# RKWin93/E2E-MAPPO-for-MT-FJSP

Measured on NVIDIA B200. Metric: MT-FJSP env-steps/sec, higher is better.
Workload: dtype f64

## Files before the change

e2e-mappo-for-mt-fjsp_b200/_lib.py:

```python
from __future__ import annotations

import ctypes as C
import os
import subprocess

_HERE = os.path.dirname(os.path.abspath(__file__))
SRC_DIR = os.path.join(_HERE, "csrc")
LIB_PATH = os.environ.get("MTFJSP_LIB") or os.path.join(_HERE, "libmtfjsp_b200.so")
HEADER = os.path.join(os.path.dirname(_HERE), "include", "mtfjsp.h")
SOURCES = ["mtfjsp_env.cu", "mtfjsp_encoder.cu", "mtfjsp_gemm.cu"]
NVCC_FLAGS = ["-gencode", "arch=compute_100a,code=sm_100a", "-O3", "-lineinfo", "-std=c++17", "-Xcompiler", "-fPIC"]
EXTRA_FLAGS = {"mtfjsp_env.cu": ["-fmad=false"]}


def _stale() -> bool:
    if not os.path.exists(LIB_PATH):
        return True
    mt = os.path.getmtime(LIB_PATH)
    deps = [os.path.join(SRC_DIR, s) for s in os.listdir(SRC_DIR)] + [HEADER, os.path.abspath(__file__)]
    return any(os.path.getmtime(d) > mt for d in deps)


def build(force: bool = False, verbose: bool = False) -> str:
    if force or _stale():
# ... 51 lines not shown
    "mtfjsp_enc_mach_proj": ([_VP, _VP, _VP, _VP, _VP, C.c_int64, _VP], _I),
    "mtfjsp_enc_gat_attend": ([_VP, _VP, _VP, _VP, C.c_int64, _I, _VP], _I),
    "mtfjsp_enc_gat_attend_bwd": ([_VP, _VP, _VP, _VP, _VP, _VP, C.c_int64, _I, _VP], _I),
    "mtfjsp_enc_gat_attend_bwd_blocks": ([C.c_int64], _I),
    "mtfjsp_enc_bias_tanh": ([_VP, _VP, C.c_int64, _I, C.c_int64, _VP], _I),
    "mtfjsp_enc_tanh_dot": ([_VP, _VP, _VP, _VP, C.c_int64, _VP], _I),
    "mtfjsp_enc_gat_trunk_tf32": ([_VP, _VP, _VP, _VP, _VP, _VP, _VP, _VP, _VP, C.c_int64, _VP], _I),
    "mtfjsp_enc_aggregate_linear_tf32": ([_VP, C.c_int64, _I, _VP, _VP, _VP, _VP, _VP, _VP, _I, _VP, _VP, _VP], _I),
    "mtfjsp_enc_select": ([_VP, _VP, _VP, C.c_float, _I, C.c_int64, _I, _U64, _VP, _I, _VP, _VP, _VP, _VP, _VP], _I),
    "mtfjsp_enc_head_tf32": ([_VP, _VP, C.c_int64, _I, _I, _VP, _VP, _I, _VP, _VP, C.c_int64, _VP, _VP, _VP, _VP, _VP, _VP], _I),
    "mtfjsp_enc_wgrad_tf32": ([_VP, _VP, C.c_int64, _I, _VP, _VP, _VP, _VP], _I),
    "mtfjsp_enc_wgrad_workspace_floats": ([_I], C.c_int64),
    "mtfjsp_enc_bn_finalize": ([_VP, C.c_int64, _VP, _VP, C.c_float, _VP, _VP, _I, _VP], _I),
    "mtfjsp_gae4": ([_VP, _VP, _VP, _VP, _VP, _VP, _I, C.c_int64, C.c_float, C.c_float, _VP], _I),
    "mtfjsp_adv_normalize": ([_VP, _VP, C.c_double, _I, C.c_int64, _VP], _I),
    "mtfjsp_launch_count": ([_VP], C.c_int64),
    "mtfjsp_bytes_per_step": ([_VP, _I], C.c_int64),
    "mtfjsp_bytes_per_random_step": ([_VP, _I], C.c_int64),
    "mtfjsp_random_step_is_fused": ([_VP], _I),
    "mtfjsp_last_error": ([], C.c_char_p),
    "mtfjsp_version": ([], C.c_char_p),
}


def lib():
    global _lib
    if _lib is None:
        if not os.path.exists(LIB_PATH):
            raise RuntimeError(
                "CUDA extension %s is missing; run `python -c 'import __graft_entry__ as g; g.build()'` "
# ... 17 lines not shown
```

e2e-mappo-for-mt-fjsp_b200/csrc/mtfjsp_env.cu:

```cuda
#include <assert.h>
#include <cuda_runtime.h>
#include <math.h>
#include <stdint.h>
#include <stdio.h>
#include <stdlib.h>
#include <string.h>

#include <new>
#include <vector>

#include "../../include/mtfjsp.h"

#define MAX_LEAVES 64
#define MAX_PROG 128
#define FULL 0xffffffffu

namespace {

struct Layout {
    int B, J, M, N, E, left_shift;
    int sd_stride, si_stride, xs_stride;
    int o_st, o_ft, o_dur, o_psel, o_scal, o_macc, o_w, o_eacc, o_eleaf, o_ipre, nich, o_sc;
    int o_mach, o_ord, o_rpred, o_cnt, o_misc, o_nxt;
    int o_mind, o_minpt, o_tt;
// ... 38 lines not shown
    unsigned char* rec;
    int rec_stride;
    int b0, b1;
    int rev;
    void* tfea;
    void* mfea;
    float* adj_w;
    int16_t* adj_src;
    uint8_t* jmask;
    int32_t* cand;
    int mask_mode;
    int obs_inc;
    uint8_t* jm_fin;
    uint8_t* jm_esa;
    int32_t* cand_int;
};

enum { MODE_STEP = 1, MODE_OBS = 2, MODE_RESET = 4, MODE_POLICY = 8,
       MODE_HOST = 16,
       MODE_FROM_RESET = 32 };

#define INFO6_PUT(b_, k_, v_)                                                                               \
    do {                                                                                                    \
        if (P.info6) P.info6[(size_t)(b_) * 6 + (k_)] = (v_);                                               \
        if (P.rec) {                                                                                        \
            unsigned char* r_ = P.rec + (size_t)(b_) * P.rec_stride;                                        \
            if ((k_) == 1) r_[REC_DONE] = (v_) != 0.0 ? 1 : 0;                                              \
            else reinterpret_cast<double*>(r_)[(k_) == 0 ? 0 : (k_) - 1] = (v_);                            \
        }                                                                                                   \
    } while (0)
// ... 580 lines not shown
#define MTFJSP_SPEC_TTG 0
#endif
    static constexpr bool TTG = MTFJSP_SPEC_TTG && !NOTT && G_ == 8 && minb(NPT_CHUNK, 0) > minb(NPT_FULL, BTT_FULL) &&
                                minb(NPT_CHUNK, 0) > minb(NPT_CHUNK, BTT_FULL);
    static constexpr int B_TT = TTG ? 0 : BTT_FULL;
    static constexpr bool CHUNK = COLD_ || TTG || minb(NPT_CHUNK, B_TT) > minb(NPT_FULL, B_TT);
    static constexpr int NPT = CHUNK ? NPT_CHUNK : NPT_FULL;
    static_assert(NPT >= 3 * M, "the random-step mode parks three compacted machine rows in the idle-term scratch");
    static constexpr int B_PT = NPT * 8;
    static constexpr int RAW = calign(B_SD + B_TT + B_PT + B_SI, 16);
    static constexpr int ENV_BYTES = env_bytes(NPT, B_TT);
    static constexpr bool BAR_IN_PAD = ENV_BYTES - RAW >= 8;
    static constexpr int ITER = (N + G - 1) / G;
    static constexpr unsigned GMASK = (G_ == 32) ? 0xffffffffu : ((1u << G_) - 1u);
    static constexpr int MINB = minb(NPT, B_TT);
};

__device__ __forceinline__ void bulk_g2s(void* smem_dst, const void* gmem_src, uint32_t bytes, uint32_t bar) {
    const uint32_t d = (uint32_t)__cvta_generic_to_shared(smem_dst);
    asm volatile("cp.async.bulk.shared::cluster.global.mbarrier::complete_tx::bytes [%0], [%1], %2, [%3];" ::"r"(d),
                 "l"(gmem_src), "r"(bytes), "r"(bar)
                 : "memory");
}

template <int G>
__device__ __forceinline__ double gmax_d(double v) {
#pragma unroll
    for (int o = G / 2; o > 0; o >>= 1) v = fmax(v, __shfl_xor_sync(FULL, v, o));
    return v;
}
// ... 32 lines not shown
        double r = 0.0;
        for (int i = 0; i < n; i++) r += a[i];
        return r;
    }
    double r[8];
    for (int i = 0; i < 8; i++) r[i] = a[i];
    int nb = n - (n & 7), i;
    for (i = 8; i < nb; i += 8)
        for (int k = 0; k < 8; k++) r[k] += a[i + k];
    double res = ((r[0] + r[1]) + (r[2] + r[3])) + ((r[4] + r[5]) + (r[6] + r[7]));
    for (; i < n; i++) res += a[i];
    return res;
}

__device__ __forceinline__ int kth_set_bit(unsigned bits, int k, int ) { return (int)__fns(bits, 0u, k + 1); }

template <class S, int MODE, typename OutT>
__global__ void __launch_bounds__(S::WARPS * 32, S::MINB) env_kernel_s(const __grid_constant__ Params P) {
    constexpr int J = S::J, M = S::M, N = S::N, G = S::G, EPW = S::EPW, ITER = S::ITER;
    extern __shared__ __align__(16) unsigned char smem_raw[];
    const int lane = threadIdx.x & 31, warp = threadIdx.x >> 5;
    const int gl = lane & (G - 1), ge = lane / G;
    const unsigned gmask = S::GMASK << (ge * G);
    const int B = P.b1;
    const int blk = P.rev ? (int)(gridDim.x - 1 - blockIdx.x) : (int)blockIdx.x;
    const int wb0 = P.b0 + (blk * S::WARPS + warp) * EPW;
    if (wb0 >= B) return;
    const int b = wb0 + ge;
    const bool active = b < B;
    const int bc = active ? b : wb0;

    unsigned char* base = smem_raw + (size_t)(warp * EPW + ge) * S::ENV_BYTES;
    double* s_sd = reinterpret_cast<double*>(base);
    const double* __restrict__ s_tt = reinterpret_cast<const double*>(base + S::B_SD);
    double* __restrict__ s_pt = reinterpret_cast<double*>(base + S::B_SD + S::B_TT);
    int16_t* __restrict__ s_si = reinterpret_cast<int16_t*>(base + S::B_SD + S::B_TT + S::B_PT);
    constexpr int RECW = rec_bytes(J) / 8, MBYTES = (J + 7) / 8;
    static_assert(6 + RECW - 5 <= S::NPT, "step info and record tail are staged in the idle-term scratch");
    unsigned char* const s_rec = reinterpret_cast<unsigned char*>(s_pt + 6) - REC_DONE;
    constexpr bool REC_STAGED = (MODE & MODE_HOST) != 0;
#define INFO6_S(k_, v_)                                                                      \
// ... 14 lines not shown
    const double* g_xs = P.xs + (size_t)bc * S::XS;
    constexpr bool fr = (MODE & MODE_FROM_RESET) != 0;
    static_assert(!fr || (!S::COLD && (MODE & MODE_STEP)), "COLD reads dur / psel from the state record, not the snapshot");
#ifdef MTFJSP_DEBUG_BOUNDS
    if (fr) assert(bc < P.L.B && P.L.sd_stride == S::SD && P.L.si_stride == S::SI);
#endif
    const double* src_sd = fr ? P.sd0 + (size_t)bc * S::SD : g_sd;
    const int16_t* src_si = fr ? P.si0 + (size_t)bc * S::SI : g_si;

    int a = 0, m = 0;
    bool sel = false;
    int cj = 0;
    int nsel_step = 0;
    int eid = 0;
    if constexpr ((MODE & MODE_POLICY) != 0) {
        const uint8_t* jsrc = (P.mask_mode == MTFJSP_MASK_ESA ? P.jm_esa : P.jm_fin) + (size_t)bc * J;
        if (gl < J) {
            sel = fr ? true : jsrc[gl] == 0;
            cj = fr ? gl * M : P.cand_int[(size_t)bc * J + gl];
        }
        if (gl < M && P.mfea1 != nullptr) eid = __ldg(P.edge_id + (size_t)bc * M + gl);
        nsel_step = fr ? 0 : g_si[S::O_MISC + 2];
    } else if (MODE & MODE_STEP) {
        if (P.act2) { const int2 am = __ldg(P.act2 + bc); a = am.x; m = am.y; }
        else { a = __ldg(P.op + bc); m = __ldg(P.mach + bc); }
    }
    uint64_t* s_bar = S::BAR_IN_PAD
                          ? reinterpret_cast<uint64_t*>(smem_raw + (size_t)(warp * EPW) * S::ENV_BYTES + S::RAW)
                          : reinterpret_cast<uint64_t*>(smem_raw + (size_t)S::WARPS * EPW * S::ENV_BYTES) + warp;
    const uint32_t bar = (uint32_t)__cvta_generic_to_shared(s_bar);
    if (lane == 0) {
        asm volatile("mbarrier.init.shared::cta.b64 [%0], 1;" ::"r"(bar));
        asm volatile("fence.mbarrier_init.release.cluster;" ::: "memory");
        asm volatile("mbarrier.arrive.expect_tx.shared::cta.b64 _, [%0], %1;" ::"r"(bar),
                     "r"((uint32_t)(EPW * (S::SM_SD * 8 + S::B_TT + S::SI * 2 + (fr ? (S::SD - (S::O_SC & ~1)) * 8 : 0))))
                     : "memory");
    }
    __syncwarp();
    if (gl == 0) {
        if constexpr (S::COLD) {
            bulk_g2s(s_sd, g_sd, S::HOT * 8, bar);
            bulk_g2s(s_sd + S::HOT, g_sd + 4 * N, S::TAILBLK * 8, bar);
        } else {
            bulk_g2s(s_sd, src_sd, S::SD * 8, bar);
        }
        if constexpr (S::B_TT > 0) bulk_g2s(base + S::B_SD, g_xs + S::O_TT, S::TT * 8, bar);
        bulk_g2s(s_si, src_si, S::SI * 2, bar);
    }
    constexpr int SC0 = S::O_SC & ~1;
    static_assert(S::NPT >= S::SD - SC0, "the scaler block is staged in the idle-term scratch");
    double wv = 0.0;
    if constexpr (fr) {
        if (gl == 0) bulk_g2s(s_pt, g_sd + SC0, (S::SD - SC0) * 8, bar);
        if (gl < 3) wv = P.weights[(size_t)bc * 3 + gl];
    }
    if constexpr (S::TTG) {
        if (gl < 4) {
            const int o = gl * 16 < M * M - 1 ? gl * 16 : M * M - 1;
            asm volatile("prefetch.global.L1 [%0];" ::"l"(g_xs + S::O_TT + o));
        }
    }
// ... 643 lines not shown
            }
            if (P.mfea && gl < M && active) emit_mach(gl, c > 0 ? (int)s_ord[incs - 1] : 0);
        }
    }

    if (fr && active) {
        const double2* s2 = reinterpret_cast<const double2*>(s_sd);
        double2* g2 = reinterpret_cast<double2*>(g_sd);
#pragma unroll 1
        for (int i = gl; i < S::SD / 2; i += G) g2[i] = s2[i];
        const int4* s4 = reinterpret_cast<const int4*>(s_si);
        int4* g4 = reinterpret_cast<int4*>(g_si);
#pragma unroll 1
        for (int i = gl; i < S::SI / 8; i += G) g4[i] = s4[i];
    }
}

__global__ void load_kernel(Layout L, const double* __restrict__ t, const double* __restrict__ p,
                            const double* __restrict__ tt, const int32_t* __restrict__ edge, int W, double* xs,
                            int8_t* edge_id) {
    size_t gid = (size_t)blockIdx.x * blockDim.x + threadIdx.x;
    size_t total = (size_t)L.B * L.N;
    if (gid < total) {
        size_t b = gid / L.N;
        int i = (int)(gid % L.N);
        const double* tr = t + gid * L.M;
        const double* pr = p + gid * L.M;
        double mn = INFINITY, mnpt = INFINITY;
        for (int m = 0; m < L.M; m++) {
            double tv = tr[m], ptv = tv * fabs(pr[m]);
// ... 447 lines not shown
    int rec_stride;
    uint8_t *dn, *inv;
    float* tmp_adj_w;
    int16_t* tmp_adj_src;
    bool loaded, reset_done, force_generic;
    bool obs_inc_enabled, obs_inc_allowed, obs_synced;
    const void* obs_ptrs[4];
    int obs_dtype;
    int host_zerocopy;
    int host_chunks, fuse_policy;
    int alternate_order, flip;
    unsigned char* slab;
    size_t slab_bytes, window_bytes;
    int l2_persist;
    int64_t launches;
    struct HostPipe* pipe;
};

struct HostPipe {
    static constexpr int MAXC = 8;
    cudaStream_t ms, cs[MAXC];
    cudaEvent_t fork, join[MAXC], hev[MAXC], kev[MAXC];
    struct Entry {
        const void* key[11];
        int mask_mode, dtype, chunks, kernels, inc;
        cudaGraphExec_t exec;
    };
    std::vector<Entry> cache;
};

// ... 6 lines not shown
static Params make_params(mtfjsp_env* h) {
    Params P;
    memset(&P, 0, sizeof P);
    P.L = h->L;
    P.pw = h->pw;
    P.sd = h->sd; P.si = h->si; P.xs = h->xs; P.t = h->t; P.p = h->p;
    P.cfgw[0] = h->cfgw[0]; P.cfgw[1] = h->cfgw[1]; P.cfgw[2] = h->cfgw[2];
    P.divisor = h->divisor; P.gamma = h->gamma;
    P.jm_fin = h->jm_fin; P.jm_esa = h->jm_esa; P.cand_int = h->cand;
    P.b0 = 0; P.b1 = h->L.B;
    return P;
}

static int flush_reset(mtfjsp_env* h, cudaStream_t s) {
    const Layout& L = h->L;
    if (h->pend_reset) {
        reset_copy_kernel<<<L.B, 128, 0, s>>>(L, h->sd0, h->si0, h->pend_w, h->sd, h->si, h->jm_fin, h->jm_esa, h->cand);
        h->launches++;
        h->pend_reset = false;
        CK(cudaGetLastError(), "reset_copy_kernel");
    }
    if (h->pend_scaler) {
        const size_t n = (size_t)L.B * 4;
        scaler_kernel<<<(unsigned)((n + 255) / 256), 256, 0, s>>>(L, h->sd, 0);
        h->launches++;
        h->pend_scaler = false;
        CK(cudaGetLastError(), "scaler_kernel");
    }
    return MTFJSP_OK;
}

static int enter(mtfjsp_env* h, cudaStream_t s, bool step = false) {
    CK(cudaSetDevice(h->device), "cudaSetDevice");
    return step ? MTFJSP_OK : flush_reset(h, s);
}

template <int MODE, typename OutT>
static int launch_env(mtfjsp_env* h, const Params& P, cudaStream_t s) {
    const Layout& L = h->L;
    int rc = flush_reset(h, s);
    if (rc != MTFJSP_OK) return rc;
    size_t smem = (size_t)L.smem_per_warp * L.warps_per_block;
    static thread_local int configured_dev = -1;
    static thread_local size_t configured_smem = 0;
    if (configured_dev != h->device || configured_smem < smem) {
        CK(cudaFuncSetAttribute(env_kernel<MODE, OutT>, cudaFuncAttributeMaxDynamicSharedMemorySize, (int)smem),
           "cudaFuncSetAttribute");
        configured_dev = h->device;
        configured_smem = smem;
    }
    int blocks = (P.b1 - P.b0 + L.warps_per_block - 1) / L.warps_per_block;
    env_kernel<MODE, OutT><<<blocks, L.warps_per_block * 32, smem, s>>>(P);
    h->launches++;
    CK(cudaGetLastError(), "env_kernel launch");
    return MTFJSP_OK;
}

template <class S, int MODE, typename OutT>
static int launch_spec(mtfjsp_env* h, const Params& P, cudaStream_t s) {
    const Layout& L = h->L;
    if (L.sd_stride != S::SD || L.si_stride != S::SI || L.xs_stride != S::XS || L.o_sc != S::O_SC || L.o_misc != S::O_MISC ||
        L.o_eacc != S::O_EACC || L.o_eleaf != S::O_ELEAF || L.o_ipre != S::O_IPRE || L.nich != S::NICH || h->pw.nleaves != S::NLEAF)
        return fail(MTFJSP_E_STATE, "specialised kernel layout mismatch");
    if constexpr (!S::COLD && (MODE & MODE_STEP) && !(MODE & (MODE_HOST | MODE_FROM_RESET))) {
        if (h->pend_reset) {
            Params Q = P;
            Q.sd0 = h->sd0; Q.si0 = h->si0; Q.weights = h->pend_w; Q.clear_ret = h->pend_scaler ? 1 : 0;
            h->pend_reset = h->pend_scaler = false;
// ... 7 lines not shown
    static const size_t extra = getenv("MTFJSP_EXTRA_SMEM") ? (size_t)atoi(getenv("MTFJSP_EXTRA_SMEM")) : 0;
    const size_t smem = (size_t)S::WARPS * S::EPW * S::ENV_BYTES + (S::BAR_IN_PAD ? 0 : 16 * ((S::WARPS * 8 + 15) / 16)) + extra;
    static thread_local int configured_dev = -1;
    if (configured_dev != h->device) {
        CK(cudaFuncSetAttribute(env_kernel_s<S, MODE, OutT>, cudaFuncAttributeMaxDynamicSharedMemorySize, (int)smem),
           "cudaFuncSetAttribute");
        configured_dev = h->device;
    }
    const int per_block = S::WARPS * S::EPW;
    const int blocks = (P.b1 - P.b0 + per_block - 1) / per_block;
    Params Q = P;
    if (h->alternate_order && (MODE & MODE_STEP)) {
        Q.rev = h->flip;
        h->flip ^= 1;
    }
    if (h->window_bytes && (MODE & MODE_STEP)) {
        cudaLaunchConfig_t cfg = {};
        cfg.gridDim = dim3(blocks);
        cfg.blockDim = dim3(S::WARPS * 32);
        cfg.dynamicSmemBytes = smem;
        cfg.stream = s;
        cudaLaunchAttribute at[1];
        at[0].id = cudaLaunchAttributeAccessPolicyWindow;
        at[0].val.accessPolicyWindow.base_ptr = h->slab;
        at[0].val.accessPolicyWindow.num_bytes = h->window_bytes;
        at[0].val.accessPolicyWindow.hitRatio = 1.0f;
        at[0].val.accessPolicyWindow.hitProp = cudaAccessPropertyPersisting;
        at[0].val.accessPolicyWindow.missProp = cudaAccessPropertyStreaming;
        cfg.attrs = at;
        cfg.numAttrs = 1;
        CK(cudaLaunchKernelEx(&cfg, env_kernel_s<S, MODE, OutT>, Q), "env_kernel_s launch");
    } else {
        env_kernel_s<S, MODE, OutT><<<blocks, S::WARPS * 32, smem, s>>>(Q);
    }
    h->launches++;
    CK(cudaGetLastError(), "env_kernel_s launch");
    return MTFJSP_OK;
}

#define MTFJSP_SPEC_SIZES(X) \
    X(6, 6, 8, 4, false) X(10, 6, 16, 1, false) X(20, 6, 32, 1, false) X(10, 10, 16, 1, false) X(15, 10, 32, 1, true) \
    X(20, 10, 32, 1, true) X(30, 20, 32, 1, true)

static int envs_per_wave(int J, int M, int device) {
    int sms = 0;
    if (cudaDeviceGetAttribute(&sms, cudaDevAttrMultiProcessorCount, device) != cudaSuccess || sms <= 0) return 0;
#define X(JJ, MM, GG, WW, CC) \
    if (J == JJ && M == MM) return sms * Spec<JJ, MM, GG, WW, CC>::MINB * WW * Spec<JJ, MM, GG, WW, CC>::EPW;
    MTFJSP_SPEC_SIZES(X)
#undef X
    return 0;
// ... 141 lines not shown
    L.smem_per_warp = align_up(off, 16);
    int wpb = 8;
    while (wpb > 1 && (size_t)wpb * L.smem_per_warp > 200 * 1024) wpb >>= 1;
    if ((size_t)wpb * L.smem_per_warp > 227 * 1024) { delete h; return fail(MTFJSP_E_ARG, "instance too large for shared memory"); }
    L.warps_per_block = wpb;
    h->device = device;
    {
        const char* fg = getenv("MTFJSP_FORCE_GENERIC");
        h->force_generic = fg && fg[0] == '1';
        h->host_chunks = getenv("MTFJSP_HOST_CHUNKS") ? atoi(getenv("MTFJSP_HOST_CHUNKS")) : 4;
        h->host_zerocopy = getenv("MTFJSP_HOST_ZEROCOPY") ? atoi(getenv("MTFJSP_HOST_ZEROCOPY")) : (B >= 16384 ? 2 : 1);
        h->fuse_policy = getenv("MTFJSP_FUSE_POLICY") ? atoi(getenv("MTFJSP_FUSE_POLICY")) : 1;
        h->alternate_order = getenv("MTFJSP_ALTERNATE_ORDER") ? atoi(getenv("MTFJSP_ALTERNATE_ORDER")) : 1;
        h->obs_inc_allowed = !(getenv("MTFJSP_OBS_INCREMENTAL") && atoi(getenv("MTFJSP_OBS_INCREMENTAL")) == 0);
        h->fused_reset = getenv("MTFJSP_FUSED_RESET") ? atoi(getenv("MTFJSP_FUSED_RESET")) : 1;
    }
    h->cfgw[0] = 0.4; h->cfgw[1] = 0.4; h->cfgw[2] = 0.2; h->divisor = 1.0; h->gamma = 0.99;
    size_t Bs = (size_t)B;
#define ALLOC(ptr, bytes)                                                      \
    do {                                                                       \
        cudaError_t e_ = cudaMalloc((void**)&(ptr), (bytes));                  \
        if (e_ != cudaSuccess) { mtfjsp_destroy(h); return fail(MTFJSP_E_CUDA, "cudaMalloc", e_); } \
        cudaMemset((ptr), 0, (bytes));                                         \
    } while (0)
    ALLOC(h->sd, Bs * L.sd_stride * 8);
    {
        auto up = [](size_t x) { return (x + 255) / 256 * 256; };
        const size_t b_si = up(Bs * L.si_stride * 2), b_jm = up(Bs * J), b_cd = up(Bs * J * 4), b_xs = up(Bs * L.xs_stride * 8);
        h->slab_bytes = b_si + 2 * b_jm + b_cd + b_xs;
        ALLOC(h->slab, h->slab_bytes);
// ... 23 lines not shown
    ALLOC(h->edge_id, Bs * M);
    ALLOC(h->a_op, Bs * 4);
    ALLOC(h->a_mach, Bs * 4);
    ALLOC(h->r5, Bs * 5 * 8);
    ALLOC(h->s4, Bs * 4 * 8);
    ALLOC(h->info6, Bs * 6 * 8);
    h->rec_stride = rec_bytes(J);
    ALLOC(h->act2, Bs * 8);
    ALLOC(h->rec, Bs * h->rec_stride);
    ALLOC(h->dn, Bs);
    ALLOC(h->inv, Bs);
    ALLOC(h->tmp_adj_w, Bs * N * 2 * 4);
    ALLOC(h->tmp_adj_src, Bs * N * 2);
    ALLOC(h->sd0, Bs * L.sd_stride * 8);
    ALLOC(h->si0, Bs * L.si_stride * 2);
#undef ALLOC
    *out = h;
    return MTFJSP_OK;
}

int mtfjsp_destroy(mtfjsp_env* h) {
    if (!h) return MTFJSP_OK;
    cudaSetDevice(h->device);
    void* ptrs[] = {h->sd, h->slab, h->t, h->p, h->edge_id, h->a_op, h->a_mach,
                    h->r5, h->s4, h->info6, h->dn, h->inv, h->tmp_adj_w, h->tmp_adj_src, h->act2, h->rec, h->sd0, h->si0};
    for (void* q : ptrs)
        if (q) cudaFree(q);
    if (h->pipe) {
        for (auto& e : h->pipe->cache) cudaGraphExecDestroy(e.exec);
        cudaStreamDestroy(h->pipe->ms);
        cudaEventDestroy(h->pipe->fork);
        for (int c = 0; c < HostPipe::MAXC; c++) {
            cudaStreamDestroy(h->pipe->cs[c]); cudaEventDestroy(h->pipe->join[c]);
            cudaEventDestroy(h->pipe->hev[c]); cudaEventDestroy(h->pipe->kev[c]);
        }
        delete h->pipe;
    }
    delete h;
    return MTFJSP_OK;
}

int mtfjsp_set_params(mtfjsp_env* h, double w_mk, double w_ec, double w_tt, double scaling_divisor, double gamma) {
// ... 509 lines not shown
    return host_step_impl(h, io, task_fea, mach_fea, adj_w, adj_src, mask_mode, dtype, (cudaStream_t)stream);
}

int mtfjsp_step_host_packed(mtfjsp_env* h, const int32_t* actions_host, void* records_host, void* task_fea, void* mach_fea,
                            float* adj_w, int16_t* adj_src, int mask_mode, int dtype, void* stream) {
    if (!h || !actions_host || !records_host) return fail(MTFJSP_E_ARG, "mtfjsp_step_host_packed: bad argument");
    if (!h->reset_done) return fail(MTFJSP_E_STATE, "mtfjsp_step_host_packed before mtfjsp_reset");
    int rc = enter(h, (cudaStream_t)stream);
    if (rc) return rc;
    HostIO io = {nullptr, nullptr, actions_host, nullptr, nullptr, nullptr, (unsigned char*)records_host};
    return host_step_impl(h, io, task_fea, mach_fea, adj_w, adj_src, mask_mode, dtype, (cudaStream_t)stream);
}

int mtfjsp_host_record_bytes(const mtfjsp_env* h) { return h ? h->rec_stride : 0; }

int64_t mtfjsp_launch_count(const mtfjsp_env* h) { return h ? h->launches : 0; }

int64_t mtfjsp_bytes_per_step(const mtfjsp_env* h, int dtype) {
    if (!h) return 0;
    const int64_t N = h->L.N, M = h->L.M, J = h->L.J;
    int64_t b_state = 18 * N + 42 * M + 8 * J + (N + 7) / 8 + 160;
    int64_t fe = dtype == MTFJSP_F64 ? 8 : 4;
    int64_t b_out = 12 * fe * N + 18 * N + 8 * fe * M + 5 * J + 41;
    return 8 + 2 * b_state + b_out;
}

int64_t mtfjsp_bytes_per_random_step(const mtfjsp_env* h, int dtype) {
    if (!h) return 0;
    const int64_t M = h->L.M, J = h->L.J;
    const int64_t fe = dtype == MTFJSP_F64 ? 8 : 4;
// ... 10 lines not shown
```

e2e-mappo-for-mt-fjsp_b200/env.py:

```python
from __future__ import annotations

import ctypes as C

import numpy as np
import torch

from . import _lib
from ._lib import check

F32, F64 = 0, 1
MASK_FINISHED, MASK_ESA = 0, 1


def _ptr(t):
    return None if t is None else C.c_void_p(t.data_ptr())


def _stream():
    return C.c_void_p(torch.cuda.current_stream().cuda_stream)


def _to_dev(x, device, dtype):
    if not torch.is_tensor(x):
        x = torch.as_tensor(np.ascontiguousarray(x))
# ... 192 lines not shown
        return dict(mach=mach, st=st, ft=ft, routes=routes)

    def export_scaler(self):
        dev, B = self.device, self.B
        R = torch.empty((B, 4), dtype=torch.float64, device=dev)
        mean = torch.empty_like(R)
        S = torch.empty_like(R)
        n = torch.empty((B,), dtype=torch.int64, device=dev)
        check(self._lib.mtfjsp_export_scaler(self._h, _ptr(R), _ptr(mean), _ptr(S), _ptr(n), _stream()), "mtfjsp_export_scaler")
        return dict(R=R, mean=mean, S=S, n=n)

    @property
    def launch_count(self):
        return int(self._lib.mtfjsp_launch_count(self._h))

    def bytes_per_step(self):
        return int(self._lib.mtfjsp_bytes_per_step(self._h, self._dt))

    def bytes_per_random_step(self):
        return int(self._lib.mtfjsp_bytes_per_random_step(self._h, self._dt))

    @property
    def random_step_is_fused(self):
        return bool(self._lib.mtfjsp_random_step_is_fused(self._h))
```

e2e-mappo-for-mt-fjsp_b200/parallel_env.py:

```python
from __future__ import annotations

import random

import numpy as np
import torch

from .env import MASK_ESA, MASK_FINISHED, BatchedMTFJSPEnv


def draw_reward_weights(kind: str, configs: dict):
    if kind == "01":
        w = np.array([random.uniform(0, 1) for _ in range(3)])
        return w / np.sum(w, axis=-1)
    if kind == "0.1":
        nums = [round(random.uniform(0, 1), 1) for _ in range(3)]
        total = sum(nums)
        return np.array([round(x / total, 1) for x in nums])
    if kind == "eval":
        return np.array([configs["weight_mk"], configs["weight_ec"], configs["weight_tt"]], dtype=np.float64)
    raise ValueError("Random_weight_type must be '01', '0.1' or 'eval'")


def gantt_text(machine_routes, st, ft, n_machine, width=72):
    horizon = max([float(ft[int(t) - 1]) for r in machine_routes.values() for t in r] + [1e-9])
# ... 151 lines not shown
    def DGFJSPEnv_paral_step(self, joint_actions):
        self._flush_scaler_reset()
        if isinstance(joint_actions, (list, tuple)):
            acts = np.fromiter((v for pair in joint_actions for v in pair), dtype=np.int32, count=2 * self.batch_size)
            acts = acts.reshape(self.batch_size, 2)
        else:
            acts = np.asarray(joint_actions, dtype=np.int32).reshape(self.batch_size, 2)
        dev = self._env.device
        op = torch.as_tensor(np.ascontiguousarray(acts[:, 0])).to(dev)
        mc = torch.as_tensor(np.ascontiguousarray(acts[:, 1])).to(dev)
        self._env.step_obs(op, mc, MASK_ESA)
        self._invalidate()
        if self.compat == "ell":
            e = self._env
            info = torch.cat((e.reward5[:, :1], e.done.to(torch.float64).unsqueeze(1), e.scaled4), dim=1).cpu().numpy()
            self.oenv_info = info
            if bool(e.invalid.any()):
                print("============= 'DGFJSPEnv_paral_step': invalid (task, machine) for envs",
                      torch.nonzero(e.invalid).flatten().tolist())
            adj, mfea, tfea = self._emit_obs()
            return adj, info, mfea, tfea
        r5 = self._env.reward5.cpu().numpy()
        s4 = self._env.scaled4.cpu().numpy()
        done = self._env.done.cpu().numpy()
        inv = self._env.invalid.cpu().numpy()
        if inv.any():
            print("============= 'DGFJSPEnv_paral_step': invalid (task, machine) for envs", np.nonzero(inv)[0].tolist())
        rows = np.concatenate([r5[:, :1], done[:, None].astype(np.float64), s4], axis=1).tolist()
        for row, dn in zip(rows, done.tolist()):
            row[1] = bool(dn)
        self.oenv_info = rows
        adj, mfea, tfea = self._emit_obs()
        return adj, self.oenv_info, mfea, tfea

    def reset_data(self):
        self.paral_env_DG = []
        self.oenv_info = []

    def _emit_obs(self):
        if self.compat == "ell":
# ... 70 lines not shown
```

e2e-mappo-for-mt-fjsp_b200/single_env.py:

```python
from __future__ import annotations

import numpy as np
import torch

from .env import MASK_ESA, BatchedMTFJSPEnv
from .parallel_env import draw_reward_weights, gantt_text


class _Configs:

    def __init__(self, d):
        self.__dict__.update(d or {})


class _NodeView:

    def __init__(self, env):
        self._e = env

    def __getitem__(self, task_id):
        e = self._e
        N = e.total_tasks_without_dummies
        if task_id == 0 or task_id == N + 1:
            return {"machine": -2, "duration": 0, "scheduled": True, "start_time": 0, "finish_time": 0, "job": -1}
# ... 75 lines not shown
        self.reward_random_weight = draw_reward_weights(Random_weight_type, self._cfg)
        self._env.reset(np.asarray(self.reward_random_weight, dtype=np.float64)[None])
        self._env.obs(MASK_ESA)
        self._cache = {}
        return self._state_array()

    def step(self, joint_action):
        a, m = int(joint_action[0]), int(joint_action[1])
        self._op[0], self._mc[0] = a, m
        len_before = len(self.machine_routes[m]) if 0 <= m < self.n_machines else 0
        self._env.step_obs(self._op, self._mc, MASK_ESA)
        self._cache = {}
        r5 = self._env.reward5.cpu().numpy()[0]
        invalid = bool(self._env.invalid.cpu().numpy()[0])
        done = bool(self._env.done.cpu().numpy()[0])
        info = {"action": a}
        if invalid:
            info.update({"valid_action": False, "node_id": a + 1})
        else:
            self.selected_action.append(a)
            self.selected_action_machine.append(m)
            hs = self._host_state()
            pos = int(np.nonzero(hs["routes"][m] == a)[0][0])
            method = "_insert_at_index_0" if pos == 0 else "_append_at_the_end" if pos == len_before else "left_shift"
            info.update({"start_time": float(hs["st"][a]), "finish_time": float(hs["ft"][a]), "node_id": a + 1,
                         "valid_action": True, "scheduling_method": method, "left_shift": int(method == "left_shift")})
            self._it_s[a] = int(np.trunc(-float(r5[2])))
        info["reward_function"] = "wrk"
        state9 = self._state_array()
        res, ft_s, it_s, adj, tasks_fea3, machines_fea, tasks_fea12, _, _ = state9
# ... 88 lines not shown
```

include/mtfjsp.h:

```cpp
#ifndef MTFJSP_H
#define MTFJSP_H

#include <stdint.h>

#ifdef __cplusplus
extern "C" {
#endif

typedef struct mtfjsp_env mtfjsp_env;

enum { MTFJSP_F32 = 0, MTFJSP_F64 = 1 };
enum { MTFJSP_MASK_FINISHED = 0, MTFJSP_MASK_ESA = 1 };
enum {
    MTFJSP_OK = 0,
    MTFJSP_E_ARG = -1,
    MTFJSP_E_CUDA = -2,
    MTFJSP_E_STATE = -3
};


int mtfjsp_create(mtfjsp_env** h, int B, int J, int M, int E, int left_shift, int device);
int mtfjsp_destroy(mtfjsp_env* h);

int mtfjsp_set_params(mtfjsp_env* h, double w_mk, double w_ec, double w_tt, double scaling_divisor, double gamma);
// ... 80 lines not shown
int mtfjsp_enc_linear_tf32(const float* X, int64_t rows, int K, const float* W, const float* bias, const float* in_scale,
                           const float* in_shift, int in_relu, float* Z, double* stats, void* stream);
int mtfjsp_enc_aggregate_linear_tf32(const float* X, int64_t B, int N, const float* adj_w, const int16_t* adj_src, const float* W,
                                     const float* bias, const float* in_scale, const float* in_shift, int in_relu, float* Z,
                                     double* stats, void* stream);
int mtfjsp_enc_wgrad_tf32(const float* dY, const float* X, int64_t rows, int K, float* dW, float* db, float* workspace,
                          void* stream);
int64_t mtfjsp_enc_wgrad_workspace_floats(int K);
int mtfjsp_enc_bn_finalize(const double* stats, int64_t rows, const float* gamma, const float* beta, float eps,
                           float* scale, float* shift, int C, void* stream);

int mtfjsp_gae4(const float* r, const float* v, const float* v_next, const float* done, float* adv, double* stats, int T,
                int64_t B, float gamma, float lam, void* stream);
int mtfjsp_adv_normalize(float* adv, const double* stats, double count, int T, int64_t B, void* stream);

int64_t mtfjsp_launch_count(const mtfjsp_env* h);
int64_t mtfjsp_bytes_per_step(const mtfjsp_env* h, int dtype);
int64_t mtfjsp_bytes_per_random_step(const mtfjsp_env* h, int dtype);
int mtfjsp_random_step_is_fused(const mtfjsp_env* h);
const char* mtfjsp_last_error(void);
const char* mtfjsp_version(void);

#ifdef __cplusplus
}
#endif
#endif
```

Measured before the change: 1.029 billion.

## Overlap consecutive env step launches with PDL and per-warp epoch flags

Consecutive policy-step launches of the env kernel now use programmatic dependent launch. Each warp publishes an epoch flag with a release reduction when it finishes. The next launch starts early, prefetches the read-only transport-time table, and has each warp acquire-wait only on its own env group's flag before it loads actions and state. This is meant to hide launch latency and the kernel tail between steps, at the cost of extra global flag traffic, spin-waiting with a timeout error path, a mapped host error word, and extra host-side chain bookkeeping. It is disabled under stream capture and for partial batches.

Result: faster. 1.073 billion, median of 6 (+4.2%).

```diff
diff --git a/e2e-mappo-for-mt-fjsp_b200/_lib.py b/e2e-mappo-for-mt-fjsp_b200/_lib.py
--- a/e2e-mappo-for-mt-fjsp_b200/_lib.py
+++ b/e2e-mappo-for-mt-fjsp_b200/_lib.py
@@ -89,6 +89,7 @@
     "mtfjsp_enc_bn_finalize": ([_VP, C.c_int64, _VP, _VP, C.c_float, _VP, _VP, _I, _VP], _I),
     "mtfjsp_gae4": ([_VP, _VP, _VP, _VP, _VP, _VP, _I, C.c_int64, C.c_float, C.c_float, _VP], _I),
     "mtfjsp_adv_normalize": ([_VP, _VP, C.c_double, _I, C.c_int64, _VP], _I),
+    "mtfjsp_launch_overlap_error": ([_VP], _I),
     "mtfjsp_launch_count": ([_VP], C.c_int64),
     "mtfjsp_bytes_per_step": ([_VP, _I], C.c_int64),
     "mtfjsp_bytes_per_random_step": ([_VP, _I], C.c_int64),
diff --git a/e2e-mappo-for-mt-fjsp_b200/csrc/mtfjsp_env.cu b/e2e-mappo-for-mt-fjsp_b200/csrc/mtfjsp_env.cu
--- a/e2e-mappo-for-mt-fjsp_b200/csrc/mtfjsp_env.cu
+++ b/e2e-mappo-for-mt-fjsp_b200/csrc/mtfjsp_env.cu
@@ -76,6 +76,9 @@
     uint8_t* jm_fin;
     uint8_t* jm_esa;
     int32_t* cand_int;
+    unsigned long long* done_ep;
+    unsigned long long ep, wait_ep;
+    unsigned* ovl_err;
 };
 
 enum { MODE_STEP = 1, MODE_OBS = 2, MODE_RESET = 4, MODE_POLICY = 8,
@@ -686,6 +689,7 @@
     static constexpr int ITER = (N + G - 1) / G;
     static constexpr unsigned GMASK = (G_ == 32) ? 0xffffffffu : ((1u << G_) - 1u);
     static constexpr int MINB = minb(NPT, B_TT);
+    static constexpr bool OVL = WARPS_ > 1;
 };
 
 __device__ __forceinline__ void bulk_g2s(void* smem_dst, const void* gmem_src, uint32_t bytes, uint32_t bar) {
@@ -748,6 +752,29 @@
 }
 
 __device__ __forceinline__ int kth_set_bit(unsigned bits, int k, int ) { return (int)__fns(bits, 0u, k + 1); }
+
+__device__ __forceinline__ void ovl_wait(const unsigned long long* flag, unsigned long long want, unsigned* err) {
+    unsigned long long v;
+    asm volatile("ld.acquire.gpu.global.u64 %0, [%1];" : "=l"(v) : "l"(flag) : "memory");
+    if (v >= want) return;
+    uint64_t t0, t;
+    asm volatile("mov.u64 %0, %%globaltimer;" : "=l"(t0));
+    unsigned ns = 32;
+    do {
+        __nanosleep(ns);
+        if (ns < 1024) ns <<= 1;
+        asm volatile("ld.acquire.gpu.global.u64 %0, [%1];" : "=l"(v) : "l"(flag) : "memory");
+        asm volatile("mov.u64 %0, %%globaltimer;" : "=l"(t));
+        if (v < want && t - t0 > 1000000000ull) {
+            *(volatile unsigned*)err = 1u;
+            __threadfence_system();
+            return;
+        }
+    } while (v < want);
+}
+__device__ __forceinline__ void ovl_release(unsigned long long* flag, unsigned long long ep) {
+    asm volatile("red.release.gpu.global.max.u64 [%0], %1;" ::"l"(flag), "l"(ep) : "memory");
+}
 
 template <class S, int MODE, typename OutT>
 __global__ void __launch_bounds__(S::WARPS * 32, S::MINB) env_kernel_s(const __grid_constant__ Params P) {
@@ -759,6 +786,9 @@
     const int B = P.b1;
     const int blk = P.rev ? (int)(gridDim.x - 1 - blockIdx.x) : (int)blockIdx.x;
     const int wb0 = P.b0 + (blk * S::WARPS + warp) * EPW;
+    constexpr bool OVL = S::OVL && (MODE & MODE_STEP) && !(MODE & MODE_HOST);
+    if (OVL && P.ep) asm volatile("griddepcontrol.launch_dependents;" ::: "memory");
+    constexpr bool WAITS = OVL && (MODE & MODE_POLICY) && !(MODE & MODE_FROM_RESET);
     if (wb0 >= B) return;
     const int b = wb0 + ge;
     const bool active = b < B;
@@ -803,17 +833,22 @@
     int nsel_step = 0;
     int eid = 0;
     if constexpr ((MODE & MODE_POLICY) != 0) {
-        const uint8_t* jsrc = (P.mask_mode == MTFJSP_MASK_ESA ? P.jm_esa : P.jm_fin) + (size_t)bc * J;
-        if (gl < J) {
-            sel = fr ? true : jsrc[gl] == 0;
-            cj = fr ? gl * M : P.cand_int[(size_t)bc * J + gl];
-        }
         if (gl < M && P.mfea1 != nullptr) eid = __ldg(P.edge_id + (size_t)bc * M + gl);
-        nsel_step = fr ? 0 : g_si[S::O_MISC + 2];
-    } else if (MODE & MODE_STEP) {
-        if (P.act2) { const int2 am = __ldg(P.act2 + bc); a = am.x; m = am.y; }
-        else { a = __ldg(P.op + bc); m = __ldg(P.mach + bc); }
-    }
+    }
+    auto load_action = [&]() {
+        if constexpr ((MODE & MODE_POLICY) != 0) {
+            const uint8_t* jsrc = (P.mask_mode == MTFJSP_MASK_ESA ? P.jm_esa : P.jm_fin) + (size_t)bc * J;
+            if (gl < J) {
+                sel = fr ? true : jsrc[gl] == 0;
+                cj = fr ? gl * M : P.cand_int[(size_t)bc * J + gl];
+            }
+            nsel_step = fr ? 0 : g_si[S::O_MISC + 2];
+        } else if (MODE & MODE_STEP) {
+            if (P.act2) { const int2 am = __ldg(P.act2 + bc); a = am.x; m = am.y; }
+            else { a = __ldg(P.op + bc); m = __ldg(P.mach + bc); }
+        }
+    };
+    if constexpr (!WAITS) load_action();
     uint64_t* s_bar = S::BAR_IN_PAD
                           ? reinterpret_cast<uint64_t*>(smem_raw + (size_t)(warp * EPW) * S::ENV_BYTES + S::RAW)
                           : reinterpret_cast<uint64_t*>(smem_raw + (size_t)S::WARPS * EPW * S::ENV_BYTES) + warp;
@@ -826,6 +861,17 @@
                      : "memory");
     }
     __syncwarp();
+    if constexpr (WAITS && S::B_TT > 0) {
+        if (gl == 0) bulk_g2s(base + S::B_SD, g_xs + S::O_TT, S::TT * 8, bar);
+    }
+    if constexpr (WAITS) {
+        if (P.wait_ep) {
+            if (lane == 0) ovl_wait(P.done_ep + wb0 / EPW, P.wait_ep, P.ovl_err);
+            __syncwarp();
+            if (gl == 0) asm volatile("fence.proxy.async.global;" ::: "memory");
+        }
+        load_action();
+    }
     if (gl == 0) {
         if constexpr (S::COLD) {
             bulk_g2s(s_sd, g_sd, S::HOT * 8, bar);
@@ -833,7 +879,7 @@
         } else {
             bulk_g2s(s_sd, src_sd, S::SD * 8, bar);
         }
-        if constexpr (S::B_TT > 0) bulk_g2s(base + S::B_SD, g_xs + S::O_TT, S::TT * 8, bar);
+        if constexpr (!WAITS && S::B_TT > 0) bulk_g2s(base + S::B_SD, g_xs + S::O_TT, S::TT * 8, bar);
         bulk_g2s(s_si, src_si, S::SI * 2, bar);
     }
     constexpr int SC0 = S::O_SC & ~1;
@@ -1507,6 +1553,13 @@
 #pragma unroll 1
         for (int i = gl; i < S::SI / 8; i += G) g4[i] = s4[i];
     }
+    if (OVL && P.ep) {
+        __syncwarp();
+        if ((threadIdx.x & 31) == 0) {
+            const unsigned bk = P.rev ? gridDim.x - 1 - blockIdx.x : blockIdx.x;
+            ovl_release(P.done_ep + bk * S::WARPS + (threadIdx.x >> 5), P.ep);
+        }
+    }
 }
 
 __global__ void load_kernel(Layout L, const double* __restrict__ t, const double* __restrict__ p,
@@ -1984,6 +2037,11 @@
     size_t slab_bytes, window_bytes;
     int l2_persist;
     int64_t launches;
+    int launch_overlap;
+    bool ovl_chain;
+    unsigned long long* done_ep;
+    unsigned long long ep;
+    unsigned *ovl_err, *ovl_err_d;
     struct HostPipe* pipe;
 };
 
@@ -2020,6 +2078,7 @@
 
 static int flush_reset(mtfjsp_env* h, cudaStream_t s) {
     const Layout& L = h->L;
+    if (h->pend_reset || h->pend_scaler) h->ovl_chain = false;
     if (h->pend_reset) {
         reset_copy_kernel<<<L.B, 128, 0, s>>>(L, h->sd0, h->si0, h->pend_w, h->sd, h->si, h->jm_fin, h->jm_esa, h->cand);
         h->launches++;
@@ -2037,7 +2096,10 @@
 }
 
 static int enter(mtfjsp_env* h, cudaStream_t s, bool step = false) {
+    if (*(volatile unsigned*)h->ovl_err)
+        return fail(MTFJSP_E_CUDA, "a step launch waited more than 1 s for the previous one (launch overlap)");
     CK(cudaSetDevice(h->device), "cudaSetDevice");
+    if (!step) h->ovl_chain = false;
     return step ? MTFJSP_OK : flush_reset(h, s);
 }
 
@@ -2058,6 +2120,7 @@
     int blocks = (P.b1 - P.b0 + L.warps_per_block - 1) / L.warps_per_block;
     env_kernel<MODE, OutT><<<blocks, L.warps_per_block * 32, smem, s>>>(P);
     h->launches++;
+    h->ovl_chain = false;
     CK(cudaGetLastError(), "env_kernel launch");
     return MTFJSP_OK;
 }
@@ -2095,27 +2158,50 @@
         Q.rev = h->flip;
         h->flip ^= 1;
     }
+    bool pdl = false;
+    if (S::OVL && (MODE & MODE_STEP) && !(MODE & MODE_HOST) && P.b0 == 0 && P.b1 == L.B && h->launch_overlap) {
+        cudaStreamCaptureStatus cs = cudaStreamCaptureStatusNone;
+        if (cudaStreamIsCapturing(s, &cs) != cudaSuccess) {
+            cudaGetLastError();
+            cs = cudaStreamCaptureStatusActive;
+        }
+        if (cs == cudaStreamCaptureStatusNone) {
+            pdl = (MODE & MODE_POLICY) && !(MODE & MODE_FROM_RESET) && h->ovl_chain;
+            Q.done_ep = h->done_ep;
+            Q.ovl_err = h->ovl_err_d;
+            Q.wait_ep = pdl ? h->ep : 0;
+            Q.ep = h->ep + 1;
+        }
+    }
+    cudaLaunchConfig_t cfg = {};
+    cfg.gridDim = dim3(blocks);
+    cfg.blockDim = dim3(S::WARPS * 32);
+    cfg.dynamicSmemBytes = smem;
+    cfg.stream = s;
+    cudaLaunchAttribute at[2];
+    cfg.attrs = at;
     if (h->window_bytes && (MODE & MODE_STEP)) {
-        cudaLaunchConfig_t cfg = {};
-        cfg.gridDim = dim3(blocks);
-        cfg.blockDim = dim3(S::WARPS * 32);
-        cfg.dynamicSmemBytes = smem;
-        cfg.stream = s;
-        cudaLaunchAttribute at[1];
-        at[0].id = cudaLaunchAttributeAccessPolicyWindow;
-        at[0].val.accessPolicyWindow.base_ptr = h->slab;
-        at[0].val.accessPolicyWindow.num_bytes = h->window_bytes;
-        at[0].val.accessPolicyWindow.hitRatio = 1.0f;
-        at[0].val.accessPolicyWindow.hitProp = cudaAccessPropertyPersisting;
-        at[0].val.accessPolicyWindow.missProp = cudaAccessPropertyStreaming;
-        cfg.attrs = at;
-        cfg.numAttrs = 1;
-        CK(cudaLaunchKernelEx(&cfg, env_kernel_s<S, MODE, OutT>, Q), "env_kernel_s launch");
-    } else {
-        env_kernel_s<S, MODE, OutT><<<blocks, S::WARPS * 32, smem, s>>>(Q);
-    }
+        cudaLaunchAttribute& a = at[cfg.numAttrs++];
+        a.id = cudaLaunchAttributeAccessPolicyWindow;
+        a.val.accessPolicyWindow.base_ptr = h->slab;
+        a.val.accessPolicyWindow.num_bytes = h->window_bytes;
+        a.val.accessPolicyWindow.hitRatio = 1.0f;
+        a.val.accessPolicyWindow.hitProp = cudaAccessPropertyPersisting;
+        a.val.accessPolicyWindow.missProp = cudaAccessPropertyStreaming;
+    }
+    if (pdl) {
+        cudaLaunchAttribute& a = at[cfg.numAttrs++];
+        a.id = cudaLaunchAttributeProgrammaticStreamSerialization;
+        a.val.programmaticStreamSerializationAllowed = 1;
+    }
+    h->ovl_chain = false;
+    CK(cudaLaunchKernelEx(&cfg, env_kernel_s<S, MODE, OutT>, Q), "env_kernel_s launch");
     h->launches++;
     CK(cudaGetLastError(), "env_kernel_s launch");
+    if (Q.ep) {
+        h->ep = Q.ep;
+        h->ovl_chain = true;
+    }
     return MTFJSP_OK;
 }
 
@@ -2287,6 +2373,7 @@
         h->alternate_order = getenv("MTFJSP_ALTERNATE_ORDER") ? atoi(getenv("MTFJSP_ALTERNATE_ORDER")) : 1;
         h->obs_inc_allowed = !(getenv("MTFJSP_OBS_INCREMENTAL") && atoi(getenv("MTFJSP_OBS_INCREMENTAL")) == 0);
         h->fused_reset = getenv("MTFJSP_FUSED_RESET") ? atoi(getenv("MTFJSP_FUSED_RESET")) : 1;
+        h->launch_overlap = getenv("MTFJSP_LAUNCH_OVERLAP") ? atoi(getenv("MTFJSP_LAUNCH_OVERLAP")) : 1;
     }
     h->cfgw[0] = 0.4; h->cfgw[1] = 0.4; h->cfgw[2] = 0.2; h->divisor = 1.0; h->gamma = 0.99;
     size_t Bs = (size_t)B;
@@ -2340,7 +2427,13 @@
     ALLOC(h->tmp_adj_src, Bs * N * 2);
     ALLOC(h->sd0, Bs * L.sd_stride * 8);
     ALLOC(h->si0, Bs * L.si_stride * 2);
+    ALLOC(h->done_ep, Bs * sizeof(unsigned long long));
 #undef ALLOC
+    {
+        cudaError_t e_ = cudaHostAlloc((void**)&h->ovl_err, sizeof(unsigned), cudaHostAllocMapped);
+        if (e_ == cudaSuccess) { *h->ovl_err = 0; e_ = cudaHostGetDevicePointer((void**)&h->ovl_err_d, h->ovl_err, 0); }
+        if (e_ != cudaSuccess) { mtfjsp_destroy(h); return fail(MTFJSP_E_CUDA, "cudaHostAlloc", e_); }
+    }
     *out = h;
     return MTFJSP_OK;
 }
@@ -2349,9 +2442,10 @@
     if (!h) return MTFJSP_OK;
     cudaSetDevice(h->device);
     void* ptrs[] = {h->sd, h->slab, h->t, h->p, h->edge_id, h->a_op, h->a_mach,
-                    h->r5, h->s4, h->info6, h->dn, h->inv, h->tmp_adj_w, h->tmp_adj_src, h->act2, h->rec, h->sd0, h->si0};
+                    h->r5, h->s4, h->info6, h->dn, h->inv, h->tmp_adj_w, h->tmp_adj_src, h->act2, h->rec, h->sd0, h->si0, h->done_ep};
     for (void* q : ptrs)
         if (q) cudaFree(q);
+    if (h->ovl_err) cudaFreeHost(h->ovl_err);
     if (h->pipe) {
         for (auto& e : h->pipe->cache) cudaGraphExecDestroy(e.exec);
         cudaStreamDestroy(h->pipe->ms);
@@ -2891,6 +2985,8 @@
 
 int mtfjsp_host_record_bytes(const mtfjsp_env* h) { return h ? h->rec_stride : 0; }
 
+int mtfjsp_launch_overlap_error(const mtfjsp_env* h) { return h ? (int)*(volatile unsigned*)h->ovl_err : 0; }
+
 int64_t mtfjsp_launch_count(const mtfjsp_env* h) { return h ? h->launches : 0; }
 
 int64_t mtfjsp_bytes_per_step(const mtfjsp_env* h, int dtype) {
diff --git a/e2e-mappo-for-mt-fjsp_b200/env.py b/e2e-mappo-for-mt-fjsp_b200/env.py
--- a/e2e-mappo-for-mt-fjsp_b200/env.py
+++ b/e2e-mappo-for-mt-fjsp_b200/env.py
@@ -230,6 +230,15 @@
     def launch_count(self):
         return int(self._lib.mtfjsp_launch_count(self._h))
 
+    @property
+    def launch_overlap_error(self):
+        return int(self._lib.mtfjsp_launch_overlap_error(self._h))
+
+    def check_launch_overlap(self):
+        if self.launch_overlap_error:
+            raise _lib.MTFJSPError("a step launch waited more than 1 s for the previous one (launch overlap): "
+                                   "its results are not trustworthy")
+
     def bytes_per_step(self):
         return int(self._lib.mtfjsp_bytes_per_step(self._h, self._dt))
 
diff --git a/e2e-mappo-for-mt-fjsp_b200/parallel_env.py b/e2e-mappo-for-mt-fjsp_b200/parallel_env.py
--- a/e2e-mappo-for-mt-fjsp_b200/parallel_env.py
+++ b/e2e-mappo-for-mt-fjsp_b200/parallel_env.py
@@ -189,6 +189,7 @@
         if self.compat == "ell":
             e = self._env
             info = torch.cat((e.reward5[:, :1], e.done.to(torch.float64).unsqueeze(1), e.scaled4), dim=1).cpu().numpy()
+            e.check_launch_overlap()
             self.oenv_info = info
             if bool(e.invalid.any()):
                 print("============= 'DGFJSPEnv_paral_step': invalid (task, machine) for envs",
@@ -199,6 +200,7 @@
         s4 = self._env.scaled4.cpu().numpy()
         done = self._env.done.cpu().numpy()
         inv = self._env.invalid.cpu().numpy()
+        self._env.check_launch_overlap()
         if inv.any():
             print("============= 'DGFJSPEnv_paral_step': invalid (task, machine) for envs", np.nonzero(inv)[0].tolist())
         rows = np.concatenate([r5[:, :1], done[:, None].astype(np.float64), s4], axis=1).tolist()
diff --git a/e2e-mappo-for-mt-fjsp_b200/single_env.py b/e2e-mappo-for-mt-fjsp_b200/single_env.py
--- a/e2e-mappo-for-mt-fjsp_b200/single_env.py
+++ b/e2e-mappo-for-mt-fjsp_b200/single_env.py
@@ -113,6 +113,7 @@
         r5 = self._env.reward5.cpu().numpy()[0]
         invalid = bool(self._env.invalid.cpu().numpy()[0])
         done = bool(self._env.done.cpu().numpy()[0])
+        self._env.check_launch_overlap()
         info = {"action": a}
         if invalid:
             info.update({"valid_action": False, "node_id": a + 1})
diff --git a/include/mtfjsp.h b/include/mtfjsp.h
--- a/include/mtfjsp.h
+++ b/include/mtfjsp.h
@@ -118,6 +118,7 @@
                 int64_t B, float gamma, float lam, void* stream);
 int mtfjsp_adv_normalize(float* adv, const double* stats, double count, int T, int64_t B, void* stream);
 
+int mtfjsp_launch_overlap_error(const mtfjsp_env* h);
 int64_t mtfjsp_launch_count(const mtfjsp_env* h);
 int64_t mtfjsp_bytes_per_step(const mtfjsp_env* h, int dtype);
 int64_t mtfjsp_bytes_per_random_step(const mtfjsp_env* h, int dtype);
diff --git a/profiles/prof_launch_overlap.py b/profiles/prof_launch_overlap.py
--- /dev/null
+++ b/profiles/prof_launch_overlap.py
@@ -0,0 +1,96 @@
+import importlib
+import json
+import os
+import statistics
+import subprocess
+import sys
+
+import torch
+
+ROOT = os.path.dirname(os.path.dirname(os.path.abspath(__file__)))
+sys.path.insert(0, ROOT)
+envm = importlib.import_module("e2e-mappo-for-mt-fjsp_b200.env")
+ins = importlib.import_module("e2e-mappo-for-mt-fjsp_b200.instances")
+
+WORKLOADS = {"A": (6, 6, 2, 65536, 1002), "B": (10, 10, 3, 16384, 1003), "C": (30, 20, 5, 4096, 1004)}
+K, REPEATS, ROUNDS = 360, 15, int(os.environ.get("ROUNDS", "5"))
+SETTINGS = {"stream_order": "0", "overlap": "1"}
+
+
+def card():
+    try:
+        q = subprocess.run(["nvidia-smi", "--query-gpu=name,power.limit,clocks.max.sm", "--format=csv,noheader"],
+                           capture_output=True, text=True, timeout=30).stdout.strip()
+    except Exception as e:
+        q = "nvidia-smi failed: %r" % e
+    return {"torch_name": torch.cuda.get_device_name(0), "nvidia_smi": q}
+
+
+def make(setting, wl, d, w):
+    J, M, E, B, _ = wl
+    os.environ["MTFJSP_LAUNCH_OVERLAP"] = SETTINGS[setting]
+    env = envm.BatchedMTFJSPEnv(B, J, M, E, left_shift=True, obs_dtype=torch.float32, mask_mode=envm.MASK_ESA)
+    env.load(d["t"], d["p"], d["transT"], d["edge"])
+    env.scaler_init()
+    env.reset(w)
+    return {"env": env, "s": 0}
+
+
+def one_step(st, w):
+    env = st["env"]
+    if st["s"] == env.N:
+        env.reset(w)
+        env.scaler_reset()
+        st["s"] = 0
+    env.random_step(seed=1234, env_offset=0)
+    st["s"] += 1
+
+
+def timed_region(st, w):
+    times = []
+    for _ in range(REPEATS):
+        e0, e1 = torch.cuda.Event(enable_timing=True), torch.cuda.Event(enable_timing=True)
+        e0.record()
+        for _ in range(K):
+            one_step(st, w)
+        e1.record()
+        torch.cuda.synchronize()
+        times.append(e0.elapsed_time(e1))
+    return statistics.median(times) / K
+
+
+def main():
+    name = sys.argv[1] if len(sys.argv) > 1 else "A"
+    wl = WORKLOADS[name]
+    J, M, E, B, seed = wl
+    torch.cuda.set_device(0)
+    d = ins.synthetic_instances(0, B, J, M, E, seed)
+    w = torch.as_tensor(ins.random_weights(0, B, seed)).cuda()
+    envs = {k: make(k, wl, d, w) for k in SETTINGS}
+    for st in envs.values():
+        for _ in range(2 * J * M):
+            one_step(st, w)
+    rows = []
+    for r in range(ROUNDS):
+        for k, st in envs.items():
+            ms = timed_region(st, w)
+            rows.append({"round": r, "setting": k, "ms_per_step": ms})
+            print("%s round %d %-13s %.5f ms/step" % (name, r, k, ms), flush=True)
+    for st in envs.values():
+        assert st["env"].launch_overlap_error == 0
+    summary = {}
+    for k in SETTINGS:
+        ms = [x["ms_per_step"] for x in rows if x["setting"] == k]
+        summary[k] = {"ms_per_step_median": statistics.median(ms), "ms_per_step_min": min(ms), "ms_per_step_max": max(ms),
+                      "spread": max(ms) - min(ms), "env_steps_per_s": B / (statistics.median(ms) * 1e-3)}
+    summary["overlap"]["speedup"] = summary["stream_order"]["ms_per_step_median"] / summary["overlap"]["ms_per_step_median"]
+    out = {"card": card(), "workload": "%s: J%dM%dE%d %d envs, K=%d, median of %d regions, %d rounds" % (
+        name, J, M, E, B, K, REPEATS, ROUNDS), "summary": summary, "rows": rows}
+    print(json.dumps({"card": out["card"], "workload": out["workload"], "summary": summary}, indent=1))
+    if len(sys.argv) > 2:
+        with open(sys.argv[2], "w") as f:
+            json.dump(out, f, indent=1)
+
+
+if __name__ == "__main__":
+    main()
```
